# nv-tlabs/DefTet

Hardware: AMD Instinct MI355X
Metric: M tet-point tests/s (fwd+bwd) at res=70, 100k queries (higher is better)
Workload: dtype f32

## Files before the change

### deftet_amd/csrc/point_in_tet.hip

```cpp
#pragma clang fp contract(off)

#include <stdlib.h>

#include <algorithm>
#include <type_traits>
#include <vector>

#include "common.hpp"

namespace deftet {
namespace pit {

constexpr float kBig = 1048576.0f;
constexpr float kTau = 1.0f / 128.0f;
constexpr float kMargin = 1.0f / 64.0f;
constexpr float kWMin = 9.3132257e-10f;
constexpr int kMiss = 0x7F7F7F7F;
constexpr int kMaxG = 112;
constexpr int kMaxBins = 15 * 1024;
constexpr int kHitOverflow = -2;

constexpr int kHitPad = 64;
__host__ __device__ inline int hit_pad(int B) { return (B + kHitPad - 1) / kHitPad * kHitPad; }
__host__ __device__ inline size_t hit_cnt_off(int B, int T) { return (size_t)B * T * 2; }
__host__ __device__ inline size_t hit_list_off(int B, int T) { return (size_t)B * T * 2 + (size_t)3 * hit_pad(B); }
__host__ __device__ inline size_t hit_spill_off(int B, int T, int Q) { return (hit_list_off(B, T) + (size_t)B * Q + 3) / 4 * 4; }
constexpr int kHitSpilled = 1 << 30;
constexpr int kRecSlots = 2, kSpillSlots = 4;
constexpr int kOvfCap = 128;
__device__ __forceinline__ void note_overflow(int *counters, int nB, int b, int t)
{
    counters[b * 4 + 2] = 1;
    const int k = atomicAdd(&counters[nB * 4 + b * 4 + 2], 1);
    if (k < kOvfCap) counters[nB * 8 + b * kOvfCap + k] = t;
}

__device__ __forceinline__ void put_hit_record(int2 *hits, int4 *spill, size_t idx, const int (&hq)[kRecSlots + kSpillSlots], int n,
                                               int *counters, int nB, int b, int t)
{
    if (n > kRecSlots + kSpillSlots || (n > kRecSlots && !spill)) {
        hits[idx] = make_int2(-1, kHitOverflow);
        note_overflow(counters, nB, b, t);
        return;
    }
    if (n > kRecSlots) spill[idx] = make_int4(hq[2], hq[3], hq[4], hq[5]);
    hits[idx] = make_int2(n > kRecSlots ? (hq[0] | kHitSpilled) : hq[0], hq[1]);
}

#ifdef PIT_PHASE_TIMING
constexpr int kPhaseWaves = 1 << 17;
__device__ unsigned long long g_phase[kPhaseWaves][16];
#define PHASE_DECL                                                                                      \
    long long ph_t_ = clock64();                                                                        \
    const unsigned ph_w_ = (((unsigned)blockIdx.y * gridDim.x + blockIdx.x) * 4u + (threadIdx.x >> 6)) & (kPhaseWaves - 1)
#define PHASE_MARK(i)                                                                  \
    do {                                                                               \
        const long long ph_n_ = clock64();                                             \
        if ((threadIdx.x & 63) == 0) g_phase[ph_w_][i] += (unsigned long long)(ph_n_ - ph_t_); \
        ph_t_ = ph_n_;                                                                 \
// ... 740 lines not shown
            } else {
                v[3 * k] = v[3 * k + 1] = v[3 * k + 2] = __int_as_float(0x7FC00000);
            }
        }
    }
    template <bool NT = false>
    __device__ __forceinline__ static void get3(const Ref &r, float4 &a, float4 &bq, float4 &c)
    {
        float v[12];
        get4(r, v);
        a = make_float4(v[0], v[1], v[2], v[3]); bq = make_float4(v[4], v[5], v[6], v[7]); c = make_float4(v[8], v[9], v[10], v[11]);
    }
    __device__ __forceinline__ static void get(const Ref &r, float (&v)[12]) { get4(r, v); }
};
__global__ __launch_bounds__(256) void k_idx_check(const int4 *__restrict__ idx, long long n, unsigned V, int *bad)
{
    const long long i = (long long)blockIdx.x * blockDim.x + threadIdx.x;
    if (i >= n) return;
    const int4 c = idx[i];
    if ((unsigned)c.x >= V || (unsigned)c.y >= V || (unsigned)c.z >= V || (unsigned)c.w >= V) *bad = 1;
}

template <class TS_, bool F>
struct TetCfg {
    typedef TS_ TS;
    static constexpr bool flag = F;
};

template <class TS>
__global__ __launch_bounds__(256, PIT_WAVES) void k_tet_scan(typename TS::Arg tet, int T, int Q,
                                                  const float *__restrict__ gparam, int G, int Gx, const int *__restrict__ table,
                                                  long long cellStride, const float4 *__restrict__ sortedQ, int *result, int *counters,
                                                  int *irregT, int2 *hits, const float *__restrict__ pts,
                                                  const int *__restrict__ irregQ, int *ucount, int hpad, int4 *spill)
{
    if (ucount && blockIdx.x == 0 && __builtin_amdgcn_readfirstlane(threadIdx.x) == 0) {
        ucount[blockIdx.y] = 0;
        ucount[hpad + blockIdx.y] = 0;
        ucount[2 * hpad + blockIdx.y] = 0;
    }
    const int b = blockIdx.y;
    const int nblk = gridDim.x;
    const int per = (nblk + 7) >> 3;
    const int vb = (blockIdx.x & 7) * per + (blockIdx.x >> 3);
    const int t = vb * blockDim.x + threadIdx.x;
    if (vb >= nblk || t >= T) return;
    const TS ts(tet);
    float v[12];
    if constexpr (std::is_same<TS, DenseTets>::value) {
        const float4 *src = reinterpret_cast<const float4 *>(tet + ((size_t)b * T + t) * 12);
        float4 a = src[0], bq = src[1], c = src[2];
        v[0] = a.x; v[1] = a.y; v[2] = a.z; v[3] = a.w;
        v[4] = bq.x; v[5] = bq.y; v[6] = bq.z; v[7] = bq.w;
        v[8] = c.x; v[9] = c.y; v[10] = c.z; v[11] = c.w;
    } else {
        TS::get4(ts.at(b, T, t), v);
    }
    Planes P;
    make_planes(v, P);
    TetBox bx;
    const bool regular = classify(v, P, bx);
    int hq[kRecSlots + kSpillSlots] = {-1, -1, -1, -1, -1, -1};
    int hcnt = 0;
    if (!regular) {
        int k = atomicAdd(&counters[b * 4 + 0], 1);
        irregT[(size_t)b * T + k] = t;
        if (hits) hits[(size_t)b * T + t] = make_int2(-1, kHitOverflow);
        irregular_queries_tail(P, t, b, Q, pts, counters, irregQ, result);
        return;
    }
    const Grid g = load_grid(gparam + b * kGridWords);
    const float m = bx.w * kMargin;
// ... 178 lines not shown
    make_planes(vv, P);
    return accept(P, x, y, z) ? 1.0f : -1.0f;
}

template <class TS>
__device__ __noinline__ void irregular_tail_slow(typename TS::Arg tet, int t, int b, int T, int Q, const float *__restrict__ pts,
                                                 const int *__restrict__ counters, const int *__restrict__ irregQ, int *result)
{
    float v[12];
    TS::get(TS(tet).at(b, T, t), v);
    Planes P;
    make_planes(v, P);
    irregular_queries_tail(P, t, b, Q, pts, counters, irregQ, result);
}
template <class TS>
__device__ __forceinline__ void irregular_tail(typename TS::Arg tet, int t, int b, int T, int Q, const float *__restrict__ pts,
                                               const int *__restrict__ counters, const int *__restrict__ irregQ, int *result)
{
    if (counters[b * 4 + 1] > 0) irregular_tail_slow<TS>(tet, t, b, T, Q, pts, counters, irregQ, result);
}

#ifndef PIT_BATCH
#define PIT_BATCH 3
#endif
#if PIT_BATCH < 1 || PIT_BATCH > 4
#error "PIT_BATCH must be 1..4 (a wave-iteration may add at most four acceptances to the four-deep hit register)"
#endif
template <class C>
__global__ __launch_bounds__(256, PIT_WAVES) void k_tet_scan_slab(typename C::TS::Arg tet, int T, int Q,
                                                  const float *__restrict__ gparam, int G, int Gx, const int *__restrict__ table,
                                                  long long cellStride, const float4 *__restrict__ sortedQ, int *result, int *counters,
                                                  int *irregT, int2 *hits, const float *__restrict__ pts,
                                                  const int *__restrict__ irregQ, int *ucount, int hpad, int4 *spill,
                                                  const int *__restrict__ order)
{
    if (ucount && blockIdx.x == 0 && __builtin_amdgcn_readfirstlane(threadIdx.x) == 0) {
        ucount[blockIdx.y] = 0;
        ucount[hpad + blockIdx.y] = 0;
        ucount[2 * hpad + blockIdx.y] = 0;
    }
    typedef typename C::TS TS;
    constexpr bool ORD = C::flag;
    const int b = blockIdx.y;
    const int nblk = gridDim.x;
    const int per = (nblk + 7) >> 3;
    const int vb = (blockIdx.x & 7) * per + (blockIdx.x >> 3);
    const int pos = vb * blockDim.x + threadIdx.x;
    if (vb >= nblk || pos >= T) return;
    const int t = ORD ? order[pos] : pos;
    PHASE_DECL;
    const TS ts(tet);
    float v[12];
    TS::get4(ts.at(b, T, t), v);
    Filter F;
    TetBox bx;
    const Grid g = load_grid(gparam + b * kGridWords);
    {
        Planes P;
        make_planes(v, P);
        if (!classify(v, P, bx)) {
            int k = atomicAdd(&counters[b * 4 + 0], 1);
            irregT[(size_t)b * T + k] = t;
            if (hits) hits[(size_t)b * T + t] = make_int2(-1, kHitOverflow);
            irregular_queries_tail(P, t, b, Q, pts, counters, irregQ, result);
            return;
        }
        const float sigma = P.sv == 15u ? 1.0f : -1.0f;
        float S[3];
#pragma unroll
        for (int k = 0; k < 3; ++k) S[k] = fmaf(fmaxf(fabsf(bx.lo[k]), fabsf(bx.hi[k])), 2.0f * kErrScale, g.pe[k]);
        float emax = 0.f;
#pragma unroll
// ... 382 lines not shown
__device__ __forceinline__ float triple(const float *a, const float *b, const float *c)
{
    float x0 = b[1] * c[2] - b[2] * c[1];
    float x1 = b[2] * c[0] - b[0] * c[2];
    float x2 = b[0] * c[1] - b[1] * c[0];
    return (a[0] * x0 + a[1] * x1) + a[2] * x2;
}
__device__ __forceinline__ float4 bary_weights(const float4 t0, const float4 t1, const float4 t2, float px, float py, float pz)
{
    const float A[3] = {t0.x, t0.y, t0.z}, Bv[3] = {t0.w, t1.x, t1.y}, Cv[3] = {t1.z, t1.w, t2.x}, D[3] = {t2.y, t2.z, t2.w};
    const float pp[3] = {px, py, pz};
    float vap[3], vbp[3], vab[3], vac[3], vad[3], vbc[3], vbd[3];
#pragma unroll
    for (int k = 0; k < 3; ++k) {
        vap[k] = pp[k] - A[k]; vbp[k] = pp[k] - Bv[k];
        vab[k] = Bv[k] - A[k]; vac[k] = Cv[k] - A[k]; vad[k] = D[k] - A[k];
        vbc[k] = Cv[k] - Bv[k]; vbd[k] = D[k] - Bv[k];
    }
    const float v6 = 1.0f / triple(vab, vac, vad);
    float4 wq;
    wq.x = triple(vbp, vbd, vbc) * v6;
    wq.y = triple(vap, vac, vad) * v6;
    wq.z = triple(vap, vad, vab) * v6;
    wq.w = triple(vap, vab, vac) * v6;
    return wq;
}

template <class TS, bool ORD, int NT>
__device__ __forceinline__ void tet_scan_wave_body(typename TS::Arg tet, int T, int Q,
                                                  const float *__restrict__ gparam, int G, int Gx, const int *__restrict__ table,
                                                  long long cellStride, const float4 *__restrict__ sortedQ, int *result, int *counters,
                                                  int *irregT, int2 *hits, const float *__restrict__ pts,
                                                  const int *__restrict__ irregQ, int *ucount, int hpad, int4 *spill,
                                                  const int *__restrict__ order)
{
    constexpr int CAP = NT == 1 ? kWvCap : kWvCapPair, ROWS = NT == 1 ? kWvRows : kWvRowsPair;
    typedef WaveStageT<CAP, ROWS> Stage;
    __shared__ Stage s_w[kWvThreads / 64];
    __shared__ int s_hit[NT][kWvSlots + 2][kWvThreads];
#if PIT_PIN_SHAPES
    const int pinL = blockIdx.y * gridDim.x + blockIdx.x, pinB = gridDim.y;
#define PIT_BLK_B (pinL % pinB)
#define PIT_BLK_X (pinL / pinB)
#else
#define PIT_BLK_B blockIdx.y
#define PIT_BLK_X blockIdx.x
#endif
    if (ucount && PIT_BLK_X == 0 && __builtin_amdgcn_readfirstlane(threadIdx.x) == 0) {
        ucount[PIT_BLK_B] = 0;
        ucount[hpad + PIT_BLK_B] = 0;
        ucount[2 * hpad + PIT_BLK_B] = 0;
    }
    const int b = PIT_BLK_B, tid = threadIdx.x, lane = tid & 63;
    const TS ts(tet);
    Stage &W = s_w[tid >> 6];
    const int nblk = gridDim.x;
#if PIT_PIN_SHAPES
    const int vb = PIT_BLK_X;
#else
    const int per = (nblk + 7) >> 3;
    const int vb = (blockIdx.x & 7) * per + (blockIdx.x >> 3);
#endif
#undef PIT_BLK_B
#undef PIT_BLK_X
    const int t = vb * blockDim.x + tid;
    const bool valid = vb < nblk && t < (T + NT - 1) / NT;
    if (__builtin_amdgcn_ballot_w64(valid) == 0ull) return;
    auto tet_id = [&](int k) -> int {
        const int p = min(NT * t + k, T - 1);
        return ORD ? order[p] : p;
    };
    auto tet_exists = [&](int k) -> bool { return valid && (NT == 1 || NT * t + k < T); };
    PHASE_DECL;
    SPAN_MARK(0);
    const Grid g = load_grid(gparam + b * kGridWords);
    Filter F[NT];
    float eabsMax[NT], mrg[NT], wk[NT][3];
    bool regular[NT], works[NT];
    int cx0 = 0x7FFF, cx1 = 0, cy0 = 0x7FFF, cy1 = 0, cz0 = 0x7FFF, cz1 = 0;
#pragma unroll
    for (int k = 0; k < NT; ++k) {
        float v[12];
        TS::template get4<PIT_SCAN_TET_NT != 0>(ts.at(b, T, tet_id(k)), v);
        float mN[4][3], det;
// ... 363 lines not shown
            }
        }
    }
    PHASE_MARK(2);
    if (PIT_STOP == 5) { PIT_KEEP(slotA[0]); PIT_KEEP(pend0); PIT_KEEP(pend1); PIT_KEEP(npend); return; }
    if (!valid) return;
    int hcnt[NT];
#pragma unroll
    for (int k = 0; k < NT; ++k) hcnt[k] = (int)((slotA[k] - slot0[k]) / (unsigned)(kWvThreads * 4));
    if (PIT_DBG_PEND && npend > 0) {
        atomicAdd(&counters[gridDim.y * 4 + b * 4 + 1], npend);
        if (npend > 2) {
#pragma unroll
            for (int k = 0; k < NT; ++k)
                if (works[k]) {
                    const int te = tet_id(k);
                    hcnt[k] = exact_rescan_slots<TS>(ts.at(b, T, te), te, tb, sq, result + (size_t)b * Q, gparam + b * kGridWords, G, Gx,
                                                 &s_hit[k][0][tid]);
                }
        } else {
            for (int j = 0; j < npend; ++j) {
                const int pq = j == 0 ? pend0 : pend1;
                const int k = NT == 1 ? 0 : (pq >> 30) & 1, qi = pq & 0x3FFFFFFF;
                const int te = tet_id(k);
                const float *pp = pts + ((size_t)b * Q + qi) * 3;
                if (exact_accept<TS>(ts.at(b, T, te), pp[0], pp[1], pp[2]) > 0.f) {
                    atomicMin(&result[(size_t)b * Q + qi], te);
                    if (NT == 1 || k == 0) { s_hit[0][min(hcnt[0], kWvSlots)][tid] = qi; ++hcnt[0]; }
                    else { s_hit[NT - 1][min(hcnt[NT - 1], kWvSlots)][tid] = qi; ++hcnt[NT - 1]; }
                }
            }
        }
    }
#pragma unroll
    for (int k = 0; k < NT; ++k) {
        if (NT > 1 && !tet_exists(k)) continue;
        int te = tet_id(k);
        asm volatile("" : "+v"(te));
        if (!regular[k]) {
            irregular_tet_slow<TS>(tet, te, b, T, Q, pts, counters, irregT, irregQ, result, hits);
            continue;
        }
        int hc = hcnt[k];
        if (hc > kWvSlots) {
            const typename TS::Ref tv = ts.at(b, T, te);
            hc = exact_rescan_slots<TS>(tv, te, tb, sq, result + (size_t)b * Q, gparam + b * kGridWords, G, Gx, &s_hit[k][0][tid]);
        }
#pragma unroll 1
        for (int i = 0; i < kWvSlots; ++i) {
            if (__builtin_amdgcn_ballot_w64(hc > i) == 0ull) break;
#if PIT_PROBE_SCATTER == 0
            if (hc > i && !(PIT_PROBE_SKIP & 1)) atomic_smin_off_nh(resb, (unsigned)s_hit[k][i][tid] * 4u, te);
#else
            if (hc > i && spill) {
                const int qi = s_hit[k][i][tid];
                char *pb = reinterpret_cast<char *>(spill);
                const size_t nq = (size_t)gridDim.y * Q, iq = (size_t)b * Q + qi;
                bool win = true;
                if (PIT_PROBE_SCATTER == 1) atomic_smin_off_nh(resb, (unsigned)qi * 4u, te);
                else win = atomicMin(&result[iq], te) > te;
                if (win && PIT_PROBE_SCATTER == 3) {
                    float4 s0, s1, s2;
                    TS::get3(ts.at(b, T, te), s0, s1, s2);
                    const float *pp = pts + iq * 3;
                    *reinterpret_cast<float4 *>(pb + iq * 16) = bary_weights(s0, s1, s2, pp[0], pp[1], pp[2]);
                    *reinterpret_cast<float *>(pb + nq * 16 + iq * 4) = (float)te;
                    *reinterpret_cast<float *>(pb + nq * 20 + iq * 4) = (float)qi;
                } else if (win) {
                    *reinterpret_cast<float4 *>(pb + iq * 16) = make_float4((float)te, (float)qi, 0.25f, 0.5f);
                    *reinterpret_cast<float *>(pb + nq * 16 + iq * 4) = (float)te;
                    *reinterpret_cast<float *>(pb + nq * 20 + iq * 4) = (float)qi;
                }
            }
#endif
        }
        if (hits) {
            int h[kRecSlots + kSpillSlots];
#pragma unroll
            for (int i = 0; i < kRecSlots + kSpillSlots; ++i) h[i] = -1;
#pragma unroll
            for (int i = 0; i < kRecSlots; ++i)
                if (i < hc) h[i] = s_hit[k][i][tid];
            const bool spilled = hc > kRecSlots && hc <= kWvSlots && spill != nullptr && PIT_PROBE_SCATTER == 0;
            const bool over = hc > kRecSlots && !spilled;
            if (spilled) {
#pragma unroll
                for (int i = kRecSlots; i < kWvSlots; ++i)
                    if (i < hc) h[i] = s_hit[k][i][tid];
                spill[(size_t)b * T + te] = make_int4(h[2], h[3], h[4], h[5]);
                h[0] |= kHitSpilled;
            }
            if (over) note_overflow(counters, gridDim.y, b, te);
            if (!(PIT_PROBE_SKIP & 2)) store_rec(hits + (size_t)b * T + te, over ? make_int2(-1, kHitOverflow) : make_int2(h[0], h[1]));
        }
        irregular_tail<TS>(tet, te, b, T, Q, pts, counters, irregQ, result);
    }
    PHASE_MARK(3);
    SPAN_MARK(1);
}

#define PIT_SCAN_PARAMS                                                                                                               \
    typename C::TS::Arg tet, int T, int Q, const float *__restrict__ gparam, int G, int Gx, const int *__restrict__ table,      \
        long long cellStride, const float4 *__restrict__ sortedQ, int *result, int *counters, int *irregT, int2 *hits,                \
        const float *__restrict__ pts, const int *__restrict__ irregQ, int *ucount, int hpad, int4 *spill, const int *__restrict__ order
#define PIT_SCAN_FWD tet, T, Q, gparam, G, Gx, table, cellStride, sortedQ, result, counters, irregT, hits, pts, irregQ, ucount, hpad, spill, order
template <class C>
__global__ __launch_bounds__(kWvThreads, PIT_WAVES2) void k_tet_scan_wave(PIT_SCAN_PARAMS)
{
    tet_scan_wave_body<typename C::TS, C::flag, 1>(PIT_SCAN_FWD);
}
template <class C>
__global__ __launch_bounds__(kWvThreads, PIT_WAVES_PAIR) void k_tet_scan_pair(PIT_SCAN_PARAMS)
{
    tet_scan_wave_body<typename C::TS, C::flag, 2>(PIT_SCAN_FWD);
}
#undef PIT_SCAN_PARAMS
#undef PIT_SCAN_FWD

#ifndef PIT_FIN_QPT
#define PIT_FIN_QPT 1
#endif
template <class TS, int QPT = PIT_FIN_QPT>
__global__ __launch_bounds__(256) void k_finalize(typename TS::Arg tet, const float *__restrict__ pts, int T,
                                                  int Q, const int *__restrict__ result, float *cond, float *bary,
                                                  const float *__restrict__ pred, float *occ, const int2 *__restrict__ hits,
                                                  int *ucount, int *ulist, const int *__restrict__ counters,
                                                  const int *__restrict__ irregT, int hpad, int pin, const float *__restrict__ gparam)
{
    __shared__ int s_cnt[4], s_base;
    const int2 sb = shape_block(pin);
    const int b = sb.x;
    const TS ts(tet);
    int q[QPT], r[QPT];
    bool live[QPT];
    size_t i[QPT];
    float px[QPT], py[QPT], pz[QPT];
#pragma unroll
    for (int j = 0; j < QPT; ++j) {
// ... 401 lines not shown
                mine = q >= 0 && cond[(size_t)b * Q + q] == tLf;
                base += 64;
            }
            if (mine) {
                const size_t i = (size_t)b * Q + q;
                float G3[3];
                tet_grad_add(g, pts + i * 3, reinterpret_cast<const float4 *>(grad_w)[i], part, G3);
                if (grad_pts) { grad_pts[i * 3] = G3[0]; grad_pts[i * 3 + 1] = G3[1]; grad_pts[i * 3 + 2] = G3[2]; }
                if (want_pred) part[12] += gocc[i];
            }
            if (ordered) best = next_hit(best, false);
        }
        if (!ordered) {
#pragma unroll
            for (int k = 0; k < 13; ++k) {
                float v = part[k];
#pragma unroll
                for (int off = 32; off > 0; off >>= 1) v += __shfl_xor(v, off);
                part[k] = v;
            }
        }
        if (lane == L) {
#pragma unroll
            for (int k = 0; k < 13; ++k) park[k][tid] = part[k];
            parked = true;
        }
    }
    return parked;
}

#ifndef PIT_BWD_WAVES
#define PIT_BWD_WAVES 7
#endif
template <class C>
__global__ __launch_bounds__(256, PIT_BWD_WAVES) void k_bary_bwd_hits(typename C::TS::Arg tet, const float *__restrict__ pts,
                                                       const float *__restrict__ cond, const float *__restrict__ grad_w,
                                                       const int2 *__restrict__ hits, int T, int Q, float *grad_tet,
                                                       float *grad_pts, int accumulate, const float *__restrict__ gocc,
                                                       float *grad_pred, float *missPart, int nMissParts, int *hitWords,
                                                       const int *__restrict__ ulist, int pad, const int4 *__restrict__ spill, int pin,
                                                       unsigned long long *rowMask)
{
    __shared__ float wsum[4];
    __shared__ float s_vals[kMissStride];
    __shared__ int s_last;
    __shared__ __attribute__((aligned(16))) float s_buf[13 * 256];
    float4(*s_rows)[192] = reinterpret_cast<float4(*)[192]>(s_buf);
    float(*s_park)[256] = reinterpret_cast<float(*)[256]>(s_buf);
    typedef typename C::TS TS;
    constexpr bool SPARSE = C::flag;
    const int2 sb = shape_block(pin);
    const int b = sb.x, bx = PIT_BWD_REV ? (int)gridDim.x - 1 - sb.y : sb.y, tid = threadIdx.x, lane = tid & 63;
    const bool side = grad_pred && bx < nMissParts;
    float missPartial = 0.f;
    if (side) {
        float gm = 0.f;
        for (int q = bx * blockDim.x + tid; q < Q; q += nMissParts * blockDim.x)
            if (cond[(size_t)b * Q + q] < 0.f) gm += gocc[(size_t)b * Q + q];
#pragma unroll
        for (int off = 32; off > 0; off >>= 1) gm += __shfl_xor(gm, off);
        if (lane == 0) wsum[tid >> 6] = gm;
        __syncthreads();
        missPartial = __int_as_float(__builtin_amdgcn_readfirstlane(__float_as_int((wsum[0] + wsum[1]) + (wsum[2] + wsum[3]))));
    }
    const int t = bx * blockDim.x + tid;
    const bool live = t < T;
    int2 h = live ? stream_load(hits + (size_t)b * T + t) : make_int2(-1, -1);
    const bool spilled = h.y != kHitOverflow && h.x >= 0 && (h.x & kHitSpilled) != 0;
    if (spilled) h.x &= ~kHitSpilled;
    bool parked = false;
    const int nU = hitWords[b];
    if (nU > 0) {
        const bool anyQ = hitWords[2 * pad + b] != 0;
        const unsigned long long need = __ballot(live && (h.y == kHitOverflow || anyQ));
        if (need) parked = bwd_rescan<TS>(tet, pts, cond, grad_w, gocc, grad_pts, grad_pred != nullptr, ulist, b, T, Q, nU, need, t, s_park);
    }
    float acc[12];
#pragma unroll
    for (int k = 0; k < 12; ++k) acc[k] = 0.f;
    float gp = 0.f;
    if (h.x >= 0 && h.y != kHitOverflow) {
        TetGrad g;
        tet_grad_setup<TS>(TS(tet).at(b, T, t), g);
        unsigned hu[8] = {(unsigned)h.x, (unsigned)h.y, ~0u, ~0u, ~0u, ~0u, ~0u, ~0u};
        const float tf = (float)t;
        auto add_hit = [&](int q) {
            if (q < 0) return;
            const size_t i = (size_t)b * Q + q;
            const float c = cond[i], go = grad_pred ? gocc[i] : 0.f;
            const float pq[3] = {pts[i * 3], pts[i * 3 + 1], pts[i * 3 + 2]};
            const float4 gw = reinterpret_cast<const float4 *>(grad_w)[i];
            const bool won = c == tf;
            float G3[3], a2[12];
#pragma unroll
            for (int k = 0; k < 12; ++k) a2[k] = acc[k];
            tet_grad_add(g, pq, gw, a2, G3);
#pragma unroll
            for (int k = 0; k < 12; ++k) acc[k] = won ? a2[k] : acc[k];
            if (won && grad_pts) { grad_pts[i * 3] = G3[0]; grad_pts[i * 3 + 1] = G3[1]; grad_pts[i * 3 + 2] = G3[2]; }
            gp = won ? gp + go : gp;
        };
#define DEFTET_CSWAP(a, b) { const unsigned lo_ = min(hu[a], hu[b]), hi_ = max(hu[a], hu[b]); hu[a] = lo_; hu[b] = hi_; }
        if (!__any(spilled)) {
            DEFTET_CSWAP(0, 1)
#pragma unroll 1
            for (int k = 0; k < 2 && __any(hu[0] != ~0u); ++k) {
                add_hit((int)hu[0]);
                hu[0] = hu[1]; hu[1] = ~0u;
            }
        } else {
            if (spilled) {
                const int4 h2 = spill[(size_t)b * T + t];
                hu[2] = (unsigned)h2.x; hu[3] = (unsigned)h2.y; hu[4] = (unsigned)h2.z; hu[5] = (unsigned)h2.w;
            }
            DEFTET_CSWAP(0, 1) DEFTET_CSWAP(2, 3) DEFTET_CSWAP(4, 5) DEFTET_CSWAP(6, 7)
            DEFTET_CSWAP(0, 2) DEFTET_CSWAP(1, 3) DEFTET_CSWAP(4, 6) DEFTET_CSWAP(5, 7)
// ... 183 lines not shown
        L.chunkQ = ((Q + L.nRowBlk - 1) / L.nRowBlk + 255) / 256 * 256;
        L.bboxPart = A.take<float>((size_t)B * kBoxBlocks * 6);
        L.chunkBox = A.take<float>((size_t)B * kMaxRowBlocks * 6);
        L.irrCnt = A.take<int>((size_t)B * kMaxRowBlocks * 2);
        L.counters = A.take<int>((size_t)B * (8 + kOvfCap));
        L.gparam = A.take<float>((size_t)B * kGridWords);
        L.table = A.take<int>((size_t)B * L.cellStride);
        L.prePitch = (L.G * kSub + 1 + 31) / 32 * 32;
        L.pre = A.take<int>((size_t)B * L.nRowBlk * L.prePitch);
        L.localQ = A.take<float4>((size_t)B * Q);
        L.sortedQ = A.take<float4>((size_t)B * Q);
        L.irregT = A.take<int>((size_t)B * T);
        L.irregQ = A.take<int>((size_t)B * Q);
    }
    L.bytes = align_up(A.off, 256);
    return L;
}

}
}

using namespace deftet;
using namespace deftet::pit;

extern "C" size_t deftet_point_in_tet_workspace_bytes(int B, int T, int Q, int algo)
{
    if (B <= 0 || T < 0 || Q < 0) return 0;
    return make_layout(B, T, Q, algo, nullptr, 0).bytes;
}

extern "C" size_t deftet_point_in_tet_hits_ints(int B, int T, int Q)
{
    if (B <= 0 || T < 0 || Q < 0) return 0;
    return hit_spill_off(B, T, Q) + (size_t)B * T * 4;
}

extern "C" int deftet_point_in_tet_resolve_algo(int algo, int T, int Q) { return resolve_auto(algo, T, Q); }

extern "C" int deftet_point_in_tet_grid_dims(int T, int Q, int *G_yz, int *G_x)
{
    DEFTET_CHECK_ARG(T >= 0 && Q >= 0 && G_yz && G_x, "bad argument");
    pick_grid(T, Q, *G_yz, *G_x);
    return DEFTET_OK;
}

static int pit_check(const float *tet, const float *pts, const float *cond, const float *bary, const float *pred, const float *occ,
                     const int32_t *hit_buf, int B, int T, int Q, int algo, const void *workspace)
{
    DEFTET_CHECK_ARG(!hit_buf || (((uintptr_t)hit_buf & 15) == 0 && algo != DEFTET_PIT_BRUTE), "hit_buf must be 16-byte aligned and needs a binned algo");
    DEFTET_CHECK_ARG((pred == nullptr) == (occ == nullptr), "pred and occ must be given together");
    DEFTET_CHECK_ARG(!occ || T > 0, "paste_occ needs at least one tet");
    DEFTET_CHECK_ARG(B >= 0 && T >= 0 && Q >= 0, "negative size (B=%d T=%d Q=%d)", B, T, Q);
    DEFTET_CHECK_ARG(algo == DEFTET_PIT_AUTO || algo == DEFTET_PIT_BRUTE || algo == DEFTET_PIT_EXACT || algo == DEFTET_PIT_SLAB || algo == DEFTET_PIT_WAVE || algo == DEFTET_PIT_PAIR, "unknown algo %d", algo);
    if (T >= (1 << 24)) return set_error(DEFTET_ELIMIT, "n_tet=%d does not fit a float-encoded index (2^24)", T);
    DEFTET_CHECK_ARG(B <= 65535, "n_batch=%d exceeds the grid-y limit 65535", B);
    if (Q >= (1 << 27)) return set_error(DEFTET_ELIMIT, "n_query=%d: 16-byte query records are addressed with 32-bit byte offsets (limit 2^27)", Q);
    if (B == 0 || Q == 0) return DEFTET_OK;
    DEFTET_CHECK_ARG(pts && cond, "null pts/cond pointer");
    DEFTET_CHECK_ARG(T == 0 || tet, "null tet pointer");
    DEFTET_CHECK_ARG(((uintptr_t)tet & 15) == 0, "tet must be 16-byte aligned");
    DEFTET_CHECK_ARG(!bary || ((uintptr_t)bary & 15) == 0, "bary must be 16-byte aligned");
    DEFTET_CHECK_ARG(workspace && ((uintptr_t)workspace & 255) == 0, "workspace null or not 256-byte aligned");
    return DEFTET_OK;
}

static int pit_prepare(const Layout &L, const float *pts, int B, int Q, hipStream_t st, const float *boxIn = nullptr, float *boxOut = nullptr,
                       int32_t *missOut = nullptr)
{
    const dim3 blk(256), lblk(kLocalThreads);
    if (boxIn) {
        DEFTET_LAUNCH(k_slab_local<true>, dim3(L.nRowBlk, B), lblk, st, pts, Q, L.bboxPart, L.gparam, L.G, L.Gx, L.nRowBlk, L.prePitch, L.chunkQ,
                      L.localQ, L.pre, L.counters, L.irregQ, boxIn, L.chunkBox, L.irrCnt, L.result);
    } else {
        DEFTET_LAUNCH(k_query_bbox, dim3(kBoxBlocks, B), blk, st, pts, Q, L.bboxPart, L.counters, L.result, B, (long long)B * Q);
        DEFTET_LAUNCH(k_slab_local<false>, dim3(L.nRowBlk, B), lblk, st, pts, Q, L.bboxPart, L.gparam, L.G, L.Gx, L.nRowBlk, L.prePitch, L.chunkQ,
                      L.localQ, L.pre, L.counters, L.irregQ, (const float *)nullptr, (float *)nullptr, (int *)nullptr, (int *)nullptr);
    }
    const size_t shm = align_up((size_t)((L.G + kParts - 1) / kParts + 1) * (L.Gx | 1) * sizeof(int), 16);
    DEFTET_LAUNCH_SHM(k_slab_sort, dim3(L.G * kParts + 1, B), dim3(kSortThreads), shm, st, L.localQ, Q, L.gparam, L.G, L.Gx, L.pre, L.nRowBlk, L.prePitch,
                      L.chunkQ, L.cellStride, L.table, L.sortedQ, (size_t)Q * 16 <= ((size_t)4 << 20),
                      (const float *)(boxIn ? L.chunkBox : L.bboxPart), boxIn ? L.nRowBlk : kBoxBlocks, boxIn ? kMaxRowBlocks : kBoxBlocks, boxOut,
                      boxIn ? 1 : 0, (const int *)L.irrCnt, L.irregQ, L.counters, (int *)(boxIn ? missOut : nullptr));
    return DEFTET_OK;
}

template <class TS>
static int pit_scan(const Layout &L, typename TS::Arg tet, const float *pts, float *cond, float *bary, const float *pred, float *occ,
                    int32_t *hit_buf, int B, int T, int Q, int algo, hipStream_t st, const int32_t *order = nullptr)
{
    const dim3 blk(256);
    const dim3 gf((Q + 256 * PIT_FIN_QPT - 1) / (256 * PIT_FIN_QPT), B), gt((((T + 255) / 256 + 7) / 8) * 8, B);
    int *ucount = hit_buf ? hit_buf + hit_cnt_off(B, T) : nullptr;
    if (T > 0) {
        if (algo == DEFTET_PIT_EXACT) {
            DEFTET_LAUNCH(k_tet_scan<TS>, gt, blk, st, tet, T, Q, L.gparam, L.G, L.Gx, L.table, L.cellStride, L.sortedQ, L.result,
                          L.counters, L.irregT, (int2 *)hit_buf, pts, L.irregQ, ucount, hit_pad(B), hit_buf ? (int4 *)(hit_buf + hit_spill_off(B, T, Q)) : (int4 *)nullptr);
        } else {
            int4 *spill = hit_buf ? (int4 *)(hit_buf + hit_spill_off(B, T, Q)) : (int4 *)nullptr;
            const int kern = resolve_auto(algo, T, Q);
            const bool slab = kern == DEFTET_PIT_SLAB;
#if PIT_PROBE_SCATTER && PIT_PROBE_PREFILL
            if (spill) DEFTET_HIP(hipMemsetAsync(spill, 0, (size_t)B * Q * 24, st));
#endif
            const dim3 bw(kWvThreads);
            const dim3 gw((((T + kWvThreads - 1) / kWvThreads + 7) / 8) * 8, B);
            const dim3 gp(((((T + 1) / 2 + kWvThreads - 1) / kWvThreads + 7) / 8) * 8, B);
#define PIT_SCAN_ARGS tet, T, Q, L.gparam, L.G, L.Gx, L.table, L.cellStride, L.sortedQ, L.result, L.counters, L.irregT, (int2 *)hit_buf, pts, \
                      L.irregQ, ucount, hit_pad(B), spill, (const int *)order
            typedef TetCfg<TS, true> Ord;
            typedef TetCfg<TS, false> Plain;
            if (slab && order) DEFTET_LAUNCH(k_tet_scan_slab<Ord>, gt, blk, st, PIT_SCAN_ARGS);
            else if (slab) DEFTET_LAUNCH(k_tet_scan_slab<Plain>, gt, blk, st, PIT_SCAN_ARGS);
            else if (kern == DEFTET_PIT_PAIR && order) DEFTET_LAUNCH(k_tet_scan_pair<Ord>, gp, bw, st, PIT_SCAN_ARGS);
            else if (kern == DEFTET_PIT_PAIR) DEFTET_LAUNCH(k_tet_scan_pair<Plain>, gp, bw, st, PIT_SCAN_ARGS);
            else if (order) DEFTET_LAUNCH(k_tet_scan_wave<Ord>, gw, bw, st, PIT_SCAN_ARGS);
            else DEFTET_LAUNCH(k_tet_scan_wave<Plain>, gw, bw, st, PIT_SCAN_ARGS);
#undef PIT_SCAN_ARGS
        }
    } else if (ucount) {
        DEFTET_HIP(hipMemsetAsync(ucount, 0, (size_t)3 * hit_pad(B) * 4, st));
    }
    DEFTET_LAUNCH(k_finalize<TS>, gf, blk, st, tet, pts, T, Q, L.result, cond, bary, pred, occ, (const int2 *)hit_buf, ucount,
                  hit_buf ? hit_buf + hit_list_off(B, T) : nullptr, L.counters, L.irregT, hit_pad(B), pin_shapes(Q), (const float *)L.gparam);
    return DEFTET_OK;
}

template <class TS>
static int pit_forward_checked(typename TS::Arg tet, const float *pts, float *cond, float *bary, const float *pred, float *occ,
                               int32_t *hit_buf, int B, int T, int Q, int algo, void *workspace, size_t workspace_bytes, void *stream_,
                               const int32_t *order, const float *boxIn, float *boxOut, int32_t *missOut)
{
    Layout L = make_layout(B, T, Q, algo, workspace, workspace_bytes);
    DEFTET_CHECK_ARG(L.bytes <= workspace_bytes, "workspace too small: need %zu bytes, got %zu", L.bytes, workspace_bytes);
    hipStream_t st = as_stream(stream_);
    if (algo == DEFTET_PIT_BRUTE) {
        const dim3 blk(256), gq((Q + 255) / 256, B);
        if (T > 0) {
            long long n = (long long)B * T;
            DEFTET_LAUNCH(k_prep_records<TS>, dim3((unsigned)((n + 255) / 256)), blk, st, tet, n, L.rec, T);
        }
        DEFTET_LAUNCH(k_brute, gq, blk, st, L.rec, pts, T, Q, L.result);
        DEFTET_LAUNCH(k_finalize<TS>, dim3((Q + 256 * PIT_FIN_QPT - 1) / (256 * PIT_FIN_QPT), B), blk, st, tet, pts, T, Q, L.result, cond, bary, pred, occ, (const int2 *)nullptr, (int *)nullptr,
                      (int *)nullptr, (const int *)nullptr, L.irregT, 0, pin_shapes(Q), (const float *)nullptr);
        return DEFTET_OK;
    }
    const int rc = pit_prepare(L, pts, B, Q, st, boxIn, boxOut, missOut);
    if (rc != DEFTET_OK) return rc;
    return pit_scan<TS>(L, tet, pts, cond, bary, pred, occ, hit_buf, B, T, Q, algo, st, order);
}
static int pit_forward(const float *tet, const float *pts, float *cond, float *bary, const float *pred, float *occ, int32_t *hit_buf,
                       int B, int T, int Q, int algo, void *workspace, size_t workspace_bytes, void *stream_, const int32_t *order,
                       const float *boxIn = nullptr, float *boxOut = nullptr, int32_t *missOut = nullptr)
{
// ... 130 lines not shown
        DEFTET_HIP(hipMemcpyToSymbol(HIP_SYMBOL(deftet::pit::g_reason), z, 64));
    }
    return DEFTET_OK;
}
extern "C" int deftet_debug_phase_read(unsigned long long *out16, int reset)
{
    std::vector<unsigned long long> h((size_t)kPhaseWaves * 16);
    DEFTET_HIP(hipMemcpyFromSymbol(h.data(), HIP_SYMBOL(deftet::pit::g_phase), h.size() * sizeof(unsigned long long)));
    for (int i = 0; i < 16; ++i) out16[i] = 0;
    for (size_t w = 0; w < (size_t)kPhaseWaves; ++w)
        for (int i = 0; i < 16; ++i) out16[i] += h[w * 16 + i];
    if (reset) {
        std::fill(h.begin(), h.end(), 0ull);
        DEFTET_HIP(hipMemcpyToSymbol(HIP_SYMBOL(deftet::pit::g_phase), h.data(), h.size() * sizeof(unsigned long long)));
    }
    return DEFTET_OK;
}
#endif

constexpr long long kDenseQueriesPerTet = 2;
extern "C" size_t deftet_point_in_tet_bwd_workspace_bytes(int B, int T, int Q)
{
    if (B <= 0 || T < 0 || Q < 0) return 0;
    const size_t lists = align_up((size_t)B * T * 4, 256) + align_up((size_t)B * Q * 4, 256) + align_up((size_t)B * 4, 256);
    const size_t miss = align_up((size_t)B * kMissStride * 4, 256);
    return lists > miss ? lists : miss;
}

static bool tets_null(const float *tet) { return tet == nullptr; }
static bool tets_null(const IndexedTets &s) { return s.pos == nullptr || s.idx == nullptr; }
static bool tets_misaligned(const float *tet) { return ((uintptr_t)tet & 15) != 0; }
static bool tets_misaligned(const IndexedTets &s) { return ((uintptr_t)s.idx & 15) != 0 || ((uintptr_t)s.pos & 3) != 0; }

template <class TS>
static int pit_bwd(typename TS::Arg tet, const float *pts, const float *cond, const float *grad_w, float *grad_tet, float *grad_pts,
                   const float *grad_occ, float *grad_pred, const int32_t *hit_buf, int B, int T, int Q, int accumulate, void *workspace,
                   size_t workspace_bytes, void *stream_)
{
    DEFTET_CHECK_ARG(B >= 0 && T >= 0 && Q >= 0, "negative size");
    DEFTET_CHECK_ARG(B <= 65535, "n_batch=%d exceeds 65535", B);
    DEFTET_CHECK_ARG((grad_occ == nullptr) == (grad_pred == nullptr), "grad_occ and grad_pred must be given together");
    hipStream_t st = as_stream(stream_);
    if (B == 0) return DEFTET_OK;
    if (grad_pts && Q > 0) DEFTET_HIP(hipMemsetAsync(grad_pts, 0, (size_t)B * Q * 12, st));
    if (T == 0) return DEFTET_OK;
    DEFTET_CHECK_ARG(grad_tet && ((uintptr_t)grad_tet & 15) == 0, "grad_tet null or not 16-byte aligned");
    if (Q == 0) {
        if (!accumulate) {
            DEFTET_HIP(hipMemsetAsync(grad_tet, 0, (size_t)B * T * 48, st));
            if (grad_pred) DEFTET_HIP(hipMemsetAsync(grad_pred, 0, (size_t)B * T * 4, st));
        }
        return DEFTET_OK;
    }
    DEFTET_CHECK_ARG(!tets_null(tet) && pts && cond && grad_w, "null pointer");
    DEFTET_CHECK_ARG(!tets_misaligned(tet) && ((uintptr_t)grad_w & 15) == 0, "tet/grad_w must be 16-byte aligned");
    const bool dense = (long long)Q > kDenseQueriesPerTet * (long long)T && workspace && ((uintptr_t)workspace & 255) == 0 &&
                       workspace_bytes >= deftet_point_in_tet_bwd_workspace_bytes(B, T, Q);
    if (hit_buf && !dense) {
        DEFTET_CHECK_ARG(((uintptr_t)hit_buf & 15) == 0, "hit_buf must be 16-byte aligned");
        float *missPart = nullptr;
        if (grad_pred) {
            DEFTET_CHECK_ARG(workspace && workspace_bytes >= (size_t)B * kMissStride * 4, "workspace needed for the miss sums (80 floats per shape)");
            missPart = static_cast<float *>(workspace);
        }
        const int tblocks = (T + 255) / 256, nMissParts = tblocks < kMissParts ? tblocks : kMissParts;
        int32_t *words = const_cast<int32_t *>(hit_buf) + hit_cnt_off(B, T);
        typedef TetCfg<TS, false> Dense;
        DEFTET_LAUNCH(k_bary_bwd_hits<Dense>, dim3(tblocks, B), dim3(256), st, tet, pts, cond, grad_w, (const int2 *)hit_buf, T, Q,
                      grad_tet, grad_pts, accumulate, grad_occ, grad_pred, missPart, nMissParts, words,
                      (const int *)(hit_buf + hit_list_off(B, T)), hit_pad(B), (const int4 *)(hit_buf + hit_spill_off(B, T, Q)), pin_shapes(Q),
                      (unsigned long long *)nullptr);
    } else if (workspace) {
        const size_t need = deftet_point_in_tet_bwd_workspace_bytes(B, T, Q);
        DEFTET_CHECK_ARG(workspace_bytes >= need && ((uintptr_t)workspace & 255) == 0,
                         "backward workspace too small (%zu < %zu) or misaligned", workspace_bytes, need);
        char *w = static_cast<char *>(workspace);
        int *head = reinterpret_cast<int *>(w);
        int *next = reinterpret_cast<int *>(w + align_up((size_t)B * T * 4, 256));
        float *missSum = reinterpret_cast<float *>(w + align_up((size_t)B * T * 4, 256) + align_up((size_t)B * Q * 4, 256));
        DEFTET_HIP(hipMemsetAsync(head, 0xFF, (size_t)B * T * 4, st));
        if (grad_pred) DEFTET_HIP(hipMemsetAsync(missSum, 0, (size_t)B * 4, st));
        DEFTET_LAUNCH(k_hit_link, dim3((Q + 256 * kLinkPer - 1) / (256 * kLinkPer), B), dim3(256), st, cond, T, Q, head, next,
                      grad_occ, missSum);
        DEFTET_LAUNCH(k_bary_bwd_gather<TS>, dim3((T + 255) / 256, B), dim3(256), st, tet, pts, grad_w, head, next, T, Q,
                      grad_tet, grad_pts, accumulate, grad_occ, missSum, grad_pred);
    } else {
        if (!accumulate) DEFTET_HIP(hipMemsetAsync(grad_tet, 0, (size_t)B * T * 48, st));
        DEFTET_LAUNCH(k_bary_bwd<TS>, dim3((Q + 255) / 256, B), dim3(256), st, tet, pts, cond, grad_w, T, Q, grad_tet,
                      grad_pts);
        if (grad_pred) {
            if (!accumulate) DEFTET_HIP(hipMemsetAsync(grad_pred, 0, (size_t)B * T * 4, st));
            DEFTET_LAUNCH(k_paste_bwd, dim3((Q + 255) / 256, B), dim3(256), st, cond, grad_occ, grad_pred, T, Q);
        }
    }
    return DEFTET_OK;
}
extern "C" int deftet_point_in_tet_bwd_f32(const float *tet, const float *pts, const float *cond, const float *grad_w,
                                           float *grad_tet, float *grad_pts, const float *grad_occ, float *grad_pred,
                                           const int32_t *hit_buf, int B, int T, int Q, int accumulate, void *workspace,
                                           size_t workspace_bytes, void *stream_)
{
    return pit_bwd<DenseTets>(tet, pts, cond, grad_w, grad_tet, grad_pts, grad_occ, grad_pred, hit_buf, B, T, Q, accumulate, workspace,
                              workspace_bytes, stream_);
}
// ... 16 lines not shown
    DEFTET_CHECK_ARG((grad_occ == nullptr) == (grad_pred == nullptr), "grad_occ and grad_pred must be given together");
    DEFTET_CHECK_ARG(idx_batch == 1 || idx_batch == B, "CSR batch must be 1 or n_batch (got %d)", idx_batch);
    hipStream_t st = as_stream(stream_);
    if (B == 0) return DEFTET_OK;
    DEFTET_CHECK_ARG(V == 0 || grad_pos, "null grad_pos");
    if (T == 0 || Q == 0 || V == 0) {
        if (grad_pts && Q > 0) DEFTET_HIP(hipMemsetAsync(grad_pts, 0, (size_t)B * Q * 12, st));
        if (!accumulate) {
            if (V > 0) DEFTET_HIP(hipMemsetAsync(grad_pos, 0, (size_t)B * V * 12, st));
            if (grad_pred && T > 0) DEFTET_HIP(hipMemsetAsync(grad_pred, 0, (size_t)B * T * 4, st));
        }
        return DEFTET_OK;
    }
    DEFTET_CHECK_ARG(!tets_null(tet) && pts && cond && grad_w && csr_offsets && csr_slots, "null pointer");
    DEFTET_CHECK_ARG(!tets_misaligned(tet) && ((uintptr_t)grad_w & 15) == 0, "tet/grad_w must be 16-byte aligned");
    const size_t need = deftet_point_in_tet_bwd_to_vertices_workspace_bytes(B, T, Q);
    DEFTET_CHECK_ARG(workspace && workspace_bytes >= need && ((uintptr_t)workspace & 255) == 0,
                     "workspace null, misaligned or too small (%zu < %zu)", workspace_bytes, need);
    Arena A(workspace, workspace_bytes);
    float *rows = A.take<float>((size_t)B * T * 12);
    unsigned long long *rowMask = A.take<unsigned long long>((size_t)B * ((T + 63) / 64));
    const size_t innerBytes = deftet_point_in_tet_bwd_workspace_bytes(B, T, Q);
    void *inner = A.take<char>(innerBytes);
    const bool dense = (long long)Q > kDenseQueriesPerTet * (long long)T;
    if (hit_buf && !dense) {
        DEFTET_CHECK_ARG(((uintptr_t)hit_buf & 15) == 0, "hit_buf must be 16-byte aligned");
        if (grad_pts) DEFTET_HIP(hipMemsetAsync(grad_pts, 0, (size_t)B * Q * 12, st));
        const int tblocks = (T + 255) / 256, nMissParts = tblocks < kMissParts ? tblocks : kMissParts;
        int32_t *words = const_cast<int32_t *>(hit_buf) + hit_cnt_off(B, T);
        typedef TetCfg<TS, true> Sparse;
        DEFTET_LAUNCH(k_bary_bwd_hits<Sparse>, dim3(tblocks, B), dim3(256), st, tet, pts, cond, grad_w, (const int2 *)hit_buf, T, Q,
                      rows, grad_pts, accumulate, grad_occ, grad_pred, static_cast<float *>(inner), nMissParts, words,
                      (const int *)(hit_buf + hit_list_off(B, T)), hit_pad(B), (const int4 *)(hit_buf + hit_spill_off(B, T, Q)), pin_shapes(Q),
                      rowMask);
        return vtx::gather_bwd_rows(rows, rowMask, csr_offsets, csr_slots, grad_pos, B, V, T, idx_batch, accumulate, st);
    }
    if (accumulate) DEFTET_HIP(hipMemsetAsync(rows, 0, (size_t)B * T * 48, st));
    const int rc = pit_bwd<TS>(tet, pts, cond, grad_w, rows, grad_pts, grad_occ, grad_pred, hit_buf, B, T, Q, accumulate, inner,
                               innerBytes, stream_);
    if (rc != DEFTET_OK) return rc;
    return vtx::gather_bwd_rows(rows, nullptr, csr_offsets, csr_slots, grad_pos, B, V, T, idx_batch, accumulate, st);
}
extern "C" int deftet_point_in_tet_bwd_to_vertices_f32(const float *tet, const float *pts, const float *cond, const float *grad_w,
                                                       const float *grad_occ, const int32_t *hit_buf, const int32_t *csr_offsets,
                                                       const int32_t *csr_slots, int idx_batch, float *grad_pos, float *grad_pts,
                                                       float *grad_pred, int B, int V, int T, int Q, int accumulate, void *workspace,
                                                       size_t workspace_bytes, void *stream_)
{
    return pit_bwd_to_vertices<DenseTets>(tet, pts, cond, grad_w, grad_occ, hit_buf, csr_offsets, csr_slots, idx_batch, grad_pos, grad_pts,
                                          grad_pred, B, V, T, Q, accumulate, workspace, workspace_bytes, stream_);
}

static int pit_check_indexed(const float *pos, const int32_t *tet_idx, int idx_batch, int B, int V, int T)
{
    DEFTET_CHECK_ARG(B >= 0 && V >= 0 && T >= 0, "negative size (B=%d V=%d T=%d)", B, V, T);
    DEFTET_CHECK_ARG(idx_batch == 1 || idx_batch == B, "idx_batch must be 1 or n_batch (got %d, n_batch %d)", idx_batch, B);
    DEFTET_CHECK_ARG(((uintptr_t)tet_idx & 15) == 0, "tet_idx must be 16-byte aligned");
    DEFTET_CHECK_ARG(((uintptr_t)pos & 3) == 0, "pos must be 4-byte aligned");
    if ((long long)V * 3 >= (1ll << 31)) return set_error(DEFTET_ELIMIT, "n_vertex=%d: vertex offsets exceed 2^31", V);
    if (B > 0 && T > 0) DEFTET_CHECK_ARG(tet_idx && (pos || V == 0), "null pos/tet_idx pointer");
    return DEFTET_OK;
}
static IndexedTets make_indexed(const float *pos, const int32_t *tet_idx, int idx_batch, int V, int T)
{
    IndexedTets s;
    s.pos = pos;
    s.idx = tet_idx;
// ... 88 lines not shown
```

Baseline: 1.085 billion.

## Pack hit tets into per-wave compact buffer during forward scan for backward reuse

In the forward wave scan, tets that recorded at least one hit are packed, in wave-rank order, into a compact float4 buffer stored in the hit buffer. A per-batch flag marks whether this packing ran. The backward hit kernel then reads each hit tet's vertices from the packed rows instead of the original tet array, so each wave loads a dense block of rows rather than scattered ones. In exchange the forward pass does extra LDS staging and streaming stores, and the hit buffer grows by a full tet copy.

Result: slower. 1.032 billion (-4.9%).

```diff
diff --git a/deftet_amd/csrc/point_in_tet.hip b/deftet_amd/csrc/point_in_tet.hip
--- a/deftet_amd/csrc/point_in_tet.hip
+++ b/deftet_amd/csrc/point_in_tet.hip
@@ -25,6 +25,9 @@
 __host__ __device__ inline size_t hit_cnt_off(int B, int T) { return (size_t)B * T * 2; }
 __host__ __device__ inline size_t hit_list_off(int B, int T) { return (size_t)B * T * 2 + (size_t)3 * hit_pad(B); }
 __host__ __device__ inline size_t hit_spill_off(int B, int T, int Q) { return (hit_list_off(B, T) + (size_t)B * Q + 3) / 4 * 4; }
+__host__ __device__ inline size_t hit_t64(int T) { return ((size_t)T + 63) / 64 * 64; }
+__host__ __device__ inline size_t hit_ctet_off(int B, int T, int Q) { return hit_spill_off(B, T, Q) + (size_t)B * T * 4; }
+__host__ __device__ inline size_t hit_cflag_off(int B, int T, int Q) { return hit_ctet_off(B, T, Q) + (size_t)B * hit_t64(T) * 12; }
 constexpr int kHitSpilled = 1 << 30;
 constexpr int kRecSlots = 2, kSpillSlots = 4;
 constexpr int kOvfCap = 128;
@@ -831,12 +834,13 @@
                                                   const float *__restrict__ gparam, int G, int Gx, const int *__restrict__ table,
                                                   long long cellStride, const float4 *__restrict__ sortedQ, int *result, int *counters,
                                                   int *irregT, int2 *hits, const float *__restrict__ pts,
-                                                  const int *__restrict__ irregQ, int *ucount, int hpad, int4 *spill)
+                                                  const int *__restrict__ irregQ, int *ucount, int hpad, int4 *spill, int *cflag)
 {
     if (ucount && blockIdx.x == 0 && __builtin_amdgcn_readfirstlane(threadIdx.x) == 0) {
         ucount[blockIdx.y] = 0;
         ucount[hpad + blockIdx.y] = 0;
         ucount[2 * hpad + blockIdx.y] = 0;
+        cflag[blockIdx.y] = 0;
     }
     const int b = blockIdx.y;
     const int nblk = gridDim.x;
@@ -1081,12 +1085,13 @@
                                                   long long cellStride, const float4 *__restrict__ sortedQ, int *result, int *counters,
                                                   int *irregT, int2 *hits, const float *__restrict__ pts,
                                                   const int *__restrict__ irregQ, int *ucount, int hpad, int4 *spill,
-                                                  const int *__restrict__ order)
+                                                  const int *__restrict__ order, int *cflag)
 {
     if (ucount && blockIdx.x == 0 && __builtin_amdgcn_readfirstlane(threadIdx.x) == 0) {
         ucount[blockIdx.y] = 0;
         ucount[hpad + blockIdx.y] = 0;
         ucount[2 * hpad + blockIdx.y] = 0;
+        cflag[blockIdx.y] = 0;
     }
     typedef typename C::TS TS;
     constexpr bool ORD = C::flag;
@@ -1535,8 +1540,9 @@
                                                   long long cellStride, const float4 *__restrict__ sortedQ, int *result, int *counters,
                                                   int *irregT, int2 *hits, const float *__restrict__ pts,
                                                   const int *__restrict__ irregQ, int *ucount, int hpad, int4 *spill,
-                                                  const int *__restrict__ order)
-{
+                                                  const int *__restrict__ order, int *cflag, float4 *ctet)
+{
+    constexpr bool COMPACT = NT == 1 && !ORD && std::is_same<TS, DenseTets>::value;
     constexpr int CAP = NT == 1 ? kWvCap : kWvCapPair, ROWS = NT == 1 ? kWvRows : kWvRowsPair;
     typedef WaveStageT<CAP, ROWS> Stage;
     __shared__ Stage s_w[kWvThreads / 64];
@@ -1553,6 +1559,7 @@
         ucount[PIT_BLK_B] = 0;
         ucount[hpad + PIT_BLK_B] = 0;
         ucount[2 * hpad + PIT_BLK_B] = 0;
+        cflag[PIT_BLK_B] = COMPACT ? 1 : 0;
     }
     const int b = PIT_BLK_B, tid = threadIdx.x, lane = tid & 63;
     const TS ts(tet);
@@ -1982,6 +1989,7 @@
             }
         }
     }
+    bool has = false;
 #pragma unroll
     for (int k = 0; k < NT; ++k) {
         if (NT > 1 && !tet_exists(k)) continue;
@@ -2041,9 +2049,30 @@
                 h[0] |= kHitSpilled;
             }
             if (over) note_overflow(counters, gridDim.y, b, te);
+            has = hc > 0 && !over;
             if (!(PIT_PROBE_SKIP & 2)) store_rec(hits + (size_t)b * T + te, over ? make_int2(-1, kHitOverflow) : make_int2(h[0], h[1]));
         }
         irregular_tail<TS>(tet, te, b, T, Q, pts, counters, irregQ, result);
+    }
+    if (COMPACT && hits) {
+        static_assert(!COMPACT || CAP >= 96, "a round of 32 rows is 96 float4");
+        const lanemask_t hm = __builtin_amdgcn_ballot_w64(has);
+        if (hm != 0ull) {
+            const int rank = __popcll(hm & ((1ull << lane) - 1ull)), n = __popcll(hm);
+            float4 r0, r1, r2;
+            if (has) TS::get3(ts.at(b, T, t), r0, r1, r2);
+            float4 *dst = ctet + ((size_t)b * (size_t)((T + 63) & ~63) + (size_t)(t - lane)) * 3;
+            const int nAct = __popcll(__builtin_amdgcn_ballot_w64(true));
+            for (int base = 0; base < n; base += 32) {
+                wave_sync();
+                if (has && (unsigned)(rank - base) < 32u) {
+                    W.q[(rank - base) * 3] = r0; W.q[(rank - base) * 3 + 1] = r1; W.q[(rank - base) * 3 + 2] = r2;
+                }
+                wave_sync();
+                const int m = min(32, n - base) * 3;
+                for (int j = lane; j < m; j += nAct) stream_store(dst + base * 3 + j, W.q[j]);
+            }
+        }
     }
     PHASE_MARK(3);
     SPAN_MARK(1);
@@ -2052,8 +2081,9 @@
 #define PIT_SCAN_PARAMS                                                                                                               \
     typename C::TS::Arg tet, int T, int Q, const float *__restrict__ gparam, int G, int Gx, const int *__restrict__ table,      \
         long long cellStride, const float4 *__restrict__ sortedQ, int *result, int *counters, int *irregT, int2 *hits,                \
-        const float *__restrict__ pts, const int *__restrict__ irregQ, int *ucount, int hpad, int4 *spill, const int *__restrict__ order
-#define PIT_SCAN_FWD tet, T, Q, gparam, G, Gx, table, cellStride, sortedQ, result, counters, irregT, hits, pts, irregQ, ucount, hpad, spill, order
+        const float *__restrict__ pts, const int *__restrict__ irregQ, int *ucount, int hpad, int4 *spill, const int *__restrict__ order, \
+        int *cflag, float4 *ctet
+#define PIT_SCAN_FWD tet, T, Q, gparam, G, Gx, table, cellStride, sortedQ, result, counters, irregT, hits, pts, irregQ, ucount, hpad, spill, order, cflag, ctet
 template <class C>
 __global__ __launch_bounds__(kWvThreads, PIT_WAVES2) void k_tet_scan_wave(PIT_SCAN_PARAMS)
 {
@@ -2521,6 +2551,8 @@
 #ifndef PIT_BWD_WAVES
 #define PIT_BWD_WAVES 7
 #endif
+__device__ __forceinline__ void compact_tet_ref(const float *&r, const float *__restrict__ ctet, size_t row) { r = ctet + row * 12; }
+__device__ __forceinline__ void compact_tet_ref(IndexedTets::Ref &, const float *__restrict__, size_t) {}
 template <class C>
 __global__ __launch_bounds__(256, PIT_BWD_WAVES) void k_bary_bwd_hits(typename C::TS::Arg tet, const float *__restrict__ pts,
                                                        const float *__restrict__ cond, const float *__restrict__ grad_w,
@@ -2528,7 +2560,8 @@
                                                        float *grad_pts, int accumulate, const float *__restrict__ gocc,
                                                        float *grad_pred, float *missPart, int nMissParts, int *hitWords,
                                                        const int *__restrict__ ulist, int pad, const int4 *__restrict__ spill, int pin,
-                                                       unsigned long long *rowMask)
+                                                       unsigned long long *rowMask, const float *__restrict__ ctet,
+                                                       const int *__restrict__ cflag)
 {
     __shared__ float wsum[4];
     __shared__ float s_vals[kMissStride];
@@ -2568,9 +2601,13 @@
 #pragma unroll
     for (int k = 0; k < 12; ++k) acc[k] = 0.f;
     float gp = 0.f;
+    const bool packed = ctet != nullptr && cflag[b] != 0;
+    const lanemask_t hm = packed ? __ballot(h.x >= 0 && h.y != kHitOverflow) : 0ull;
     if (h.x >= 0 && h.y != kHitOverflow) {
         TetGrad g;
-        tet_grad_setup<TS>(TS(tet).at(b, T, t), g);
+        typename TS::Ref tr = TS(tet).at(b, T, t);
+        if (packed) compact_tet_ref(tr, ctet, (size_t)b * (size_t)((T + 63) & ~63) + (size_t)((t - lane) + __popcll(hm & ((1ull << lane) - 1ull))));
+        tet_grad_setup<TS>(tr, g);
         unsigned hu[8] = {(unsigned)h.x, (unsigned)h.y, ~0u, ~0u, ~0u, ~0u, ~0u, ~0u};
         const float tf = (float)t;
         auto add_hit = [&](int q) {
@@ -2820,7 +2857,7 @@
 extern "C" size_t deftet_point_in_tet_hits_ints(int B, int T, int Q)
 {
     if (B <= 0 || T < 0 || Q < 0) return 0;
-    return hit_spill_off(B, T, Q) + (size_t)B * T * 4;
+    return hit_cflag_off(B, T, Q) + (size_t)hit_pad(B);
 }
 
 extern "C" int deftet_point_in_tet_resolve_algo(int algo, int T, int Q) { return resolve_auto(algo, T, Q); }
@@ -2879,10 +2916,12 @@
     const dim3 blk(256);
     const dim3 gf((Q + 256 * PIT_FIN_QPT - 1) / (256 * PIT_FIN_QPT), B), gt((((T + 255) / 256 + 7) / 8) * 8, B);
     int *ucount = hit_buf ? hit_buf + hit_cnt_off(B, T) : nullptr;
+    int *cflag = hit_buf ? hit_buf + hit_cflag_off(B, T, Q) : nullptr;
     if (T > 0) {
         if (algo == DEFTET_PIT_EXACT) {
             DEFTET_LAUNCH(k_tet_scan<TS>, gt, blk, st, tet, T, Q, L.gparam, L.G, L.Gx, L.table, L.cellStride, L.sortedQ, L.result,
-                          L.counters, L.irregT, (int2 *)hit_buf, pts, L.irregQ, ucount, hit_pad(B), hit_buf ? (int4 *)(hit_buf + hit_spill_off(B, T, Q)) : (int4 *)nullptr);
+                          L.counters, L.irregT, (int2 *)hit_buf, pts, L.irregQ, ucount, hit_pad(B), hit_buf ? (int4 *)(hit_buf + hit_spill_off(B, T, Q)) : (int4 *)nullptr,
+                          cflag);
         } else {
             int4 *spill = hit_buf ? (int4 *)(hit_buf + hit_spill_off(B, T, Q)) : (int4 *)nullptr;
             const int kern = resolve_auto(algo, T, Q);
@@ -2893,20 +2932,22 @@
             const dim3 bw(kWvThreads);
             const dim3 gw((((T + kWvThreads - 1) / kWvThreads + 7) / 8) * 8, B);
             const dim3 gp(((((T + 1) / 2 + kWvThreads - 1) / kWvThreads + 7) / 8) * 8, B);
+            float4 *ctet = hit_buf ? (float4 *)(hit_buf + hit_ctet_off(B, T, Q)) : (float4 *)nullptr;
 #define PIT_SCAN_ARGS tet, T, Q, L.gparam, L.G, L.Gx, L.table, L.cellStride, L.sortedQ, L.result, L.counters, L.irregT, (int2 *)hit_buf, pts, \
-                      L.irregQ, ucount, hit_pad(B), spill, (const int *)order
+                      L.irregQ, ucount, hit_pad(B), spill, (const int *)order, cflag
             typedef TetCfg<TS, true> Ord;
             typedef TetCfg<TS, false> Plain;
             if (slab && order) DEFTET_LAUNCH(k_tet_scan_slab<Ord>, gt, blk, st, PIT_SCAN_ARGS);
             else if (slab) DEFTET_LAUNCH(k_tet_scan_slab<Plain>, gt, blk, st, PIT_SCAN_ARGS);
-            else if (kern == DEFTET_PIT_PAIR && order) DEFTET_LAUNCH(k_tet_scan_pair<Ord>, gp, bw, st, PIT_SCAN_ARGS);
-            else if (kern == DEFTET_PIT_PAIR) DEFTET_LAUNCH(k_tet_scan_pair<Plain>, gp, bw, st, PIT_SCAN_ARGS);
-            else if (order) DEFTET_LAUNCH(k_tet_scan_wave<Ord>, gw, bw, st, PIT_SCAN_ARGS);
-            else DEFTET_LAUNCH(k_tet_scan_wave<Plain>, gw, bw, st, PIT_SCAN_ARGS);
+            else if (kern == DEFTET_PIT_PAIR && order) DEFTET_LAUNCH(k_tet_scan_pair<Ord>, gp, bw, st, PIT_SCAN_ARGS, ctet);
+            else if (kern == DEFTET_PIT_PAIR) DEFTET_LAUNCH(k_tet_scan_pair<Plain>, gp, bw, st, PIT_SCAN_ARGS, ctet);
+            else if (order) DEFTET_LAUNCH(k_tet_scan_wave<Ord>, gw, bw, st, PIT_SCAN_ARGS, ctet);
+            else DEFTET_LAUNCH(k_tet_scan_wave<Plain>, gw, bw, st, PIT_SCAN_ARGS, ctet);
 #undef PIT_SCAN_ARGS
         }
     } else if (ucount) {
         DEFTET_HIP(hipMemsetAsync(ucount, 0, (size_t)3 * hit_pad(B) * 4, st));
+        DEFTET_HIP(hipMemsetAsync(cflag, 0, (size_t)hit_pad(B) * 4, st));
     }
     DEFTET_LAUNCH(k_finalize<TS>, gf, blk, st, tet, pts, T, Q, L.result, cond, bary, pred, occ, (const int2 *)hit_buf, ucount,
                   hit_buf ? hit_buf + hit_list_off(B, T) : nullptr, L.counters, L.irregT, hit_pad(B), pin_shapes(Q), (const float *)L.gparam);
@@ -3103,6 +3144,11 @@
 static bool tets_misaligned(const float *tet) { return ((uintptr_t)tet & 15) != 0; }
 static bool tets_misaligned(const IndexedTets &s) { return ((uintptr_t)s.idx & 15) != 0 || ((uintptr_t)s.pos & 3) != 0; }
 
+template <class TS>
+static const float *compact_tets(const int32_t *hit_buf, int B, int T, int Q)
+{
+    return std::is_same<TS, DenseTets>::value ? reinterpret_cast<const float *>(hit_buf + hit_ctet_off(B, T, Q)) : nullptr;
+}
 template <class TS>
 static int pit_bwd(typename TS::Arg tet, const float *pts, const float *cond, const float *grad_w, float *grad_tet, float *grad_pts,
                    const float *grad_occ, float *grad_pred, const int32_t *hit_buf, int B, int T, int Q, int accumulate, void *workspace,
@@ -3140,7 +3186,7 @@
         DEFTET_LAUNCH(k_bary_bwd_hits<Dense>, dim3(tblocks, B), dim3(256), st, tet, pts, cond, grad_w, (const int2 *)hit_buf, T, Q,
                       grad_tet, grad_pts, accumulate, grad_occ, grad_pred, missPart, nMissParts, words,
                       (const int *)(hit_buf + hit_list_off(B, T)), hit_pad(B), (const int4 *)(hit_buf + hit_spill_off(B, T, Q)), pin_shapes(Q),
-                      (unsigned long long *)nullptr);
+                      (unsigned long long *)nullptr, compact_tets<TS>(hit_buf, B, T, Q), (const int *)(hit_buf + hit_cflag_off(B, T, Q)));
     } else if (workspace) {
         const size_t need = deftet_point_in_tet_bwd_workspace_bytes(B, T, Q);
         DEFTET_CHECK_ARG(workspace_bytes >= need && ((uintptr_t)workspace & 255) == 0,
@@ -3223,7 +3269,7 @@
         DEFTET_LAUNCH(k_bary_bwd_hits<Sparse>, dim3(tblocks, B), dim3(256), st, tet, pts, cond, grad_w, (const int2 *)hit_buf, T, Q,
                       rows, grad_pts, accumulate, grad_occ, grad_pred, static_cast<float *>(inner), nMissParts, words,
                       (const int *)(hit_buf + hit_list_off(B, T)), hit_pad(B), (const int4 *)(hit_buf + hit_spill_off(B, T, Q)), pin_shapes(Q),
-                      rowMask);
+                      rowMask, compact_tets<TS>(hit_buf, B, T, Q), (const int *)(hit_buf + hit_cflag_off(B, T, Q)));
         return vtx::gather_bwd_rows(rows, rowMask, csr_offsets, csr_slots, grad_pos, B, V, T, idx_batch, accumulate, st);
     }
     if (accumulate) DEFTET_HIP(hipMemsetAsync(rows, 0, (size_t)B * T * 48, st));
```
